# uzh-rpg/rpg_svo

Measured on AMD Instinct MI355X. Metric: frames/sec sparse-align+pose-refine (VGA, 4 pyr lvls); ATE vs CPU ref, higher is better.
Workload: dtype value = default build: K1 f32 pixels/residuals/chi2/per-pixel products, f64 Jacobian rows/partials/reductions/projection/solve/pose; K4 f64 (reference-width build: roofline_f64_build.value)

## Files before the change

### include/svo_hip.h

```cpp
#ifndef SVO_HIP_H_
#define SVO_HIP_H_

#include <stddef.h>
#include <stdint.h>

#ifdef __cplusplus
extern "C" {
#endif

#define SVO_HIP_MAX_LEVELS 8
#define SVO_HIP_STORE_TAIL_PAD 256
#define SVO_HIP_MAX_PATCHES 1024

#define SVO_HIP_OK 0
#define SVO_HIP_EINVAL (-1)
#define SVO_HIP_ERANGE (-2)
#define SVO_HIP_EHIP (-3)
#define SVO_HIP_ENODEV (-4)
#define SVO_HIP_ENOMEM (-5)

#define SVO_HIP_HALFSAMPLE_SCALAR 0
#define SVO_HIP_HALFSAMPLE_SSE2 1
#define SVO_HIP_HALFSAMPLE_AUTO 2

// ... 245 lines not shown
                                       double* d_px_cur, int32_t* d_ok, int32_t* d_ref_obs, int32_t* d_search_level,
                                       double* d_A_cur_ref, uint8_t* d_patch_out, void* d_workspace,
                                       size_t workspace_bytes, void* stream);
int svo_hip_select_matches_indirect(const svo_hip_camera* cam, int M_cap, const int32_t* d_M, const int32_t* d_cell,
                                    const int32_t* d_ok, const double* d_px, const int32_t* d_level,
                                    const double* d_pos, int max_fts, int32_t* d_n, int32_t* d_sel, double* d_f,
                                    int32_t* d_level_out, double* d_pos_out, uint8_t* d_has_point, int32_t* d_signal,
                                    int32_t signal_value, void* stream);

int svo_hip_compose_poses(int n, const double* d_A, const double* d_B, double* d_out,
                          const int32_t* d_out_index, void* stream);
int svo_hip_cam2world(const svo_hip_camera* cam, int n, const double* d_px, double* d_f,
                      void* stream);
int svo_hip_frame_pose_compose(const double* d_T_cur_ref, const double* d_q_ref, const double* d_t_ref, double* d_frame_T,
                               int cur_frame, double* d_T_copy, double* d_T_out, const svo_hip_camera* cam, int n_frames,
                               int n_kf, const double* d_key_pos, const uint8_t* d_key_valid, int max_n_kfs, int32_t* d_rank,
                               int32_t* d_rank_out, int32_t* d_signal, int32_t signal_value, void* stream);

int svo_hip_pose_optimize(const svo_hip_camera* cam, int B, const int32_t* d_n, int n_stride,
                          const double* d_f, const int32_t* d_level, const double* d_pos,
                          uint8_t* d_has_point, double reproj_thresh, int n_iter,
                          double* d_T_f_w, double* d_Cov, double* d_stats, int32_t* d_ran,
                          void* stream);
int svo_hip_pose_optimize_ordered(const svo_hip_camera* cam, int B, const int32_t* d_n, int n_stride,
                                  const double* d_f, const int32_t* d_level, const double* d_pos,
                                  uint8_t* d_has_point, double reproj_thresh, int n_iter,
                                  double* d_T_f_w, double* d_Cov, double* d_stats, int32_t* d_ran,
                                  void* stream);

int svo_hip_pose_optimize_deferred(const svo_hip_camera* cam, int B, const int32_t* d_n, int n_stride,
                                   const double* d_f, const int32_t* d_level, const double* d_pos,
                                   uint8_t* d_has_point, double reproj_thresh, int n_iter, double* d_T_f_w,
                                   double* d_Cov, double* d_stats, int32_t* d_ran, void* stream);

int svo_hip_point_optimize(const svo_hip_frames* frames, int P, const int32_t* d_obs_ptr,
                           const int32_t* d_obs_frame, const double* d_obs_f, int n_iter,
                           double* d_pos, void* stream);

typedef struct svo_hip_seeds {
  float* d_a;
  float* d_b;
  float* d_mu;
  float* d_z_range;
  float* d_sigma2;
  const int32_t* d_batch_id;
} svo_hip_seeds;

#define SVO_HIP_SEED_ERASED_OLD 1
#define SVO_HIP_SEED_BEHIND 2
#define SVO_HIP_SEED_NOT_IN_FRAME 3
#define SVO_HIP_SEED_NO_MATCH 4
#define SVO_HIP_SEED_UPDATED 5
#define SVO_HIP_SEED_CONVERGED 6
#define SVO_HIP_SEED_NAN 7

typedef struct svo_hip_depth_filter_options {
  int32_t max_n_kfs;
  int32_t batch_counter;
  double seed_convergence_sigma2_thresh;
  int32_t align_1d;
  int32_t align_max_iter;
  int32_t max_epi_search_steps;
  int32_t subpix_refinement;
  int32_t epi_search_edgelet_filtering;
  int32_t n_pyr_levels;
  double epi_search_edgelet_max_angle;
// ... 204 lines not shown
```

### rpg_svo_amd/capi.py

```python
from __future__ import annotations

import ctypes as C
import os

MAX_LEVELS = 8
STORE_TAIL_PAD = 256
MAX_PATCHES = 1024

HALFSAMPLE_SCALAR, HALFSAMPLE_SSE2, HALFSAMPLE_AUTO = 0, 1, 2
SIA_STOP = 1

_LIB_PATH = os.environ.get("SVO_HIP_LIB") or os.path.join(os.path.dirname(os.path.abspath(__file__)), "lib", "libsvo_hip.so")


class SvoHipError(RuntimeError):
    pass


class PyrLayout(C.Structure):
    _fields_ = [
        ("n_levels", C.c_int32),
        ("w", C.c_int32 * MAX_LEVELS),
        ("h", C.c_int32 * MAX_LEVELS),
        ("pitch", C.c_int32 * MAX_LEVELS),
# ... 176 lines not shown
    "svo_hip_sparse_align": (_i, [C.POINTER(PyrLayout), _vp, _i, _vp, _vp, _vp, _i, _vp, _vp, _vp,
                                  C.POINTER(SiaParams), _vp, _vp, _vp, _vp, _vp, _vp, _vp, _vp]),
    "svo_hip_sparse_align_workgroup": (_i, [C.POINTER(PyrLayout), _vp, _i, _vp, _vp, _vp, _i, _vp, _vp, _vp,
                                            C.POINTER(SiaParams), _vp, _vp, _vp, _vp, _vp, _vp, _vp, _vp]),
    "svo_hip_solve6_hipsolver_workspace_bytes": (C.c_size_t, [_i]),
    "svo_hip_solve6_hipsolver": (_i, [_i, _vp, _vp, _vp, _vp, _vp, C.c_size_t, _vp]),
    "svo_hip_align_batch": (_i, [_LP, _vp, _i, _vp, _vp, _vp, _vp, _vp, _i, _vp, _vp, _vp, _vp]),
    "svo_hip_align_batch_counted": (_i, [_LP, _vp, _i, _vp, _vp, _vp, _vp, _vp, _i, _vp, _vp, _vp, _vp, _vp]),
    "svo_hip_align_workspace_bytes": (C.c_size_t, [_i]),
    "svo_hip_align_batch_phased": (_i, [_LP, _vp, _i, _vp, _vp, _vp, _vp, _vp, _i, _vp, _vp, _vp, _vp, _vp, C.c_size_t, _vp]),
    "svo_hip_update_seeds_scan_steps": (_vp, [_vp]),
    "svo_hip_update_seeds_count_evaluations": (C.c_int, [C.c_int]),
    "svo_hip_update_seeds_align_evaluations": (_vp, [_vp, C.c_int]),
    "svo_hip_match_workspace_bytes": (C.c_size_t, [_i]),
    "svo_hip_find_match_direct": (_i, [_LP, _vp, C.POINTER(Camera), C.POINTER(Frames), _i, _vp, _vp, _vp,
                                       C.POINTER(Features), _i, _i, _vp, _vp, _vp, _vp, _vp, _vp, _vp, C.c_size_t, _vp]),
    "svo_hip_reproject_map": (_i, [C.POINTER(Camera), C.POINTER(Frames), _i, _vp, C.POINTER(Map), C.POINTER(MapPatch),
                                   C.POINTER(Grid), _i, _i, _i, _i, C.POINTER(Reprojection), _vp]),
    "svo_hip_find_match_direct_indirect": (_i, [_LP, _vp, C.POINTER(Camera), C.POINTER(Frames), _i, _vp, _vp, _vp, _vp, _vp,
                                                C.POINTER(Features), _i, _i, _vp, _vp, _vp, _vp, _vp, _vp, _vp, C.c_size_t, _vp]),
    "svo_hip_select_matches_indirect": (_i, [C.POINTER(Camera), _i, _vp, _vp, _vp, _vp, _vp, _vp, _i, _vp, _vp, _vp, _vp, _vp,
                                             _vp, _vp, _i, _vp]),
    "svo_hip_reproject_points": (_i, [C.POINTER(Camera), C.POINTER(Frames), _i, _vp, _vp, _i, _i, _vp, _vp, _vp]),
    "svo_hip_compose_poses": (_i, [_i, _vp, _vp, _vp, _vp, _vp]),
    "svo_hip_frame_pose_compose": (_i, [_vp, _vp, _vp, _vp, _i, _vp, _vp, _vp, _i, _i, _vp, _vp, _i, _vp, _vp, _vp, _i, _vp]),
    "svo_hip_cam2world": (_i, [C.POINTER(Camera), _i, _vp, _vp, _vp]),
    "svo_hip_select_matches": (_i, [C.POINTER(Camera), _i, _vp, _vp, _vp, _vp, _vp, _i, _vp, _vp, _vp, _vp, _vp, _vp, _vp, _i, _vp]),
    "svo_hip_pose_optimize": (_i, [C.POINTER(Camera), _i, _vp, _i, _vp, _vp, _vp, _vp, C.c_double, _i, _vp, _vp, _vp,
                                   _vp, _vp]),
    "svo_hip_pose_optimize_ordered": (_i, [C.POINTER(Camera), _i, _vp, _i, _vp, _vp, _vp, _vp, C.c_double, _i, _vp, _vp,
                                           _vp, _vp, _vp]),
    "svo_hip_pose_optimize_deferred": (_i, [C.POINTER(Camera), _i, _vp, _i, _vp, _vp, _vp, _vp, C.c_double, _i, _vp, _vp,
                                           _vp, _vp, _vp]),
    "svo_hip_point_optimize": (_i, [C.POINTER(Frames), _i, _vp, _vp, _vp, _i, _vp, _vp]),
    "svo_hip_update_seeds": (_i, [_LP, _vp, C.POINTER(Camera), C.POINTER(Frames), _i, _vp, C.POINTER(Features),
                                  C.POINTER(Seeds), C.POINTER(DepthFilterOptions), _vp, _vp, _vp, _vp, C.c_size_t, _vp]),
    "svo_hip_seed_store_patch": (_i, [C.POINTER(SeedPatch), C.POINTER(Features), C.POINTER(Seeds), _vp]),
    "svo_hip_update_seeds_resident": (_i, [_LP, _vp, C.POINTER(Camera), C.POINTER(Frames), _i, _i, _vp, C.POINTER(Features),
                                           C.POINTER(Seeds), C.POINTER(DepthFilterOptions), _vp, _vp, _vp, _vp, _vp, C.c_size_t, _vp]),
    "svo_hip_update_seeds_resident_pose": (_i, [_LP, _vp, C.POINTER(Camera), C.POINTER(Frames), _i, _vp, _i, _vp, C.POINTER(Features),
                                                C.POINTER(Seeds), C.POINTER(DepthFilterOptions), _vp, _vp, _vp, _vp, _vp, C.c_size_t, _vp]),
    "svo_hip_find_epipolar_match_direct": (_i, [_LP, _vp, C.POINTER(Camera), C.POINTER(Frames), _i, _vp, C.POINTER(Features),
                                                _vp, _vp, _vp, C.POINTER(DepthFilterOptions), _vp, _vp, _vp, _vp, _vp, C.c_size_t, _vp]),
    "svo_hip_update_seed_batch": (_i, [_i, _vp, _vp, C.POINTER(Seeds), _vp]),
    "svo_hip_fast_workspace_bytes": (C.c_size_t, [_LP, _i, _i]),
    "svo_hip_fast_detect": (_i, [_LP, _vp, _i, _vp, _i, _i, _i, _i, _i, _vp, C.c_double, _vp, _vp, _vp, _vp, C.c_size_t, _vp]),
    "svo_hip_klt_params_default": (_i, [C.POINTER(KltParams)]),
    "svo_hip_klt_track": (_i, [_LP, _vp, _i, _vp, _vp, _i, _vp, _vp, _vp, _vp, C.POINTER(KltParams), _vp]),
    "svo_hip_klt_summarize": (_i, [C.POINTER(Camera), _i, _i, _vp, _vp, _vp, _vp, _vp, _vp, _vp, _vp]),
    "svo_hip_homography_params_default": (_i, [C.POINTER(HomographyParams)]),
    "svo_hip_homography_init": (_i, [C.POINTER(Camera), _i, _i, _vp, _vp, _vp, _vp, _vp, _vp, C.POINTER(HomographyParams),
                                     C.POINTER(HomographyOut), _vp]),
    "svo_hip_first_map": (_i, [C.POINTER(Camera), _i, _i, _vp, _vp, _vp, _vp, _vp, _vp, _vp, _vp, _vp, _i, _i, _i, _i,
                               C.POINTER(FirstMapOut), _vp]),
    "svo_hip_initialize_seeds": (_i, [C.POINTER(Camera), _i, _i, _vp, _vp, _vp, C.c_double, _vp, _vp, _vp, _i, _i,
                                      C.POINTER(SeedInitOut), _vp]),
    "svo_hip_frame_close_params_default": (_i, [C.POINTER(FrameCloseParams)]),
    "svo_hip_frame_close": (_i, [C.POINTER(Camera), _i, _i, _i, C.POINTER(FrameCloseIn), _i, _i, _i, _i, C.POINTER(FrameCloseParams),
                                 C.POINTER(FrameCloseOut), _vp]),
    "svo_hip_compute_tau_batch": (_i, [_i, _vp, _vp, _vp, C.c_double, _vp, _vp]),
}

_lib = None


def lib_path() -> str:
# ... 54 lines not shown
```

### rpg_svo_amd/csrc/pose_optimizer.hip

```cpp
#pragma clang fp contract(off)
#include "track_kernels.h"
#include "track_math.h"

using namespace svo_capi;
using namespace svo_dev;

namespace {

constexpr int PO_MINW = 4;
constexpr int PO_HALF = 32;
constexpr int PO_BLOCK = 64;
constexpr int PO_MAXN = 1024;
constexpr double SVO_EPS = 0.0000000001;

struct PoseArgs {
  Cam cam;
  const int32_t* n;
  int n_stride;
  const double* f;
  const int32_t* level;
  const double* pos;
  uint8_t* has_point;
  double reproj_thresh;
  int n_iter;
  double* T;
  double* Cov;
  double* stats;
  int32_t* ran;
  int only_flagged;
};

struct PoseLds {
  double tile[28][PO_HALF];
  unsigned long long live[PO_BLOCK / 64];
  double acc[28];
  double dT[6];
  double new_chi2;
  Se3 T, T_old;
  double scale;
  double median_d;
  double chi2;
  float median_f;
  int n_err;
  int flag;
};

__device__ __forceinline__ float tukey_weight(float x) {
  const float b_square = 4.6851f * 4.6851f;
  const float x_square = x * x;
  if (x_square <= b_square) {
    const float tmp = 1.0f - x_square / b_square;
    return tmp * tmp;
  }
  return 0.0f;
}

template <typename T>
__device__ __forceinline__ void rank_select(const T* v, int n, int k, T* out) {
  for (int i = threadIdx.x; i < n; i += PO_BLOCK) {
    const T mine = v[i];
    if (!(mine < (T)INFINITY)) continue;
    int rank = 0;
#pragma unroll 8
    for (int j = 0; j < n; ++j) {
      const T o = v[j];
      rank += (o < mine || (o == mine && j < i)) ? 1 : 0;
    }
    if (rank == k) *out = mine;
  }
}

struct PoseDyn {
  double* vals;
  float* err;
  uint8_t* hp;
};

__global__ void __launch_bounds__(PO_BLOCK, PO_MINW) pose_opt_kernel(const PoseArgs a) {
  __shared__ PoseLds s;
  SVO_DYNAMIC_LDS(double, po_dyn);
  const int ns8 = (a.n_stride + 7) & ~7;
  PoseDyn d;
  d.vals = po_dyn;
  d.err = reinterpret_cast<float*>(po_dyn + ns8);
  d.hp = reinterpret_cast<uint8_t*>(d.err + ns8);
  const int b = blockIdx.x;
  const int tid = threadIdx.x;
  if (a.only_flagged && a.ran[b] != 2) return;
  int n = a.n[b];
  n = n < 0 ? 0 : (n > a.n_stride ? a.n_stride : n);
  const size_t base = (size_t)b * a.n_stride;
  const double focal = fabs(a.cam.fx);

  if (tid == 0) {
    se3_from_Rt(a.T + 12 * b, s.T);
    s.T_old = s.T;
    s.n_err = 0;
    s.flag = 0;
    s.chi2 = 0.0;
  }
  for (int i = tid; i < n; i += PO_BLOCK) d.hp[i] = a.has_point[base + i];
  __syncthreads();
  {
    const Se3 T = s.T;
    int cnt = 0;
    for (int i = tid; i < n; i += PO_BLOCK) {
      d.err[i] = INFINITY;
      if (!d.hp[i]) continue;
      const double p[3] = {a.pos[3 * (base + i)], a.pos[3 * (base + i) + 1], a.pos[3 * (base + i) + 2]};
      const double fb[3] = {a.f[3 * (base + i)], a.f[3 * (base + i) + 1], a.f[3 * (base + i) + 2]};
      double pf[3], u0[2], u1[2];
      se3_apply(T, p, pf);
      project2d(fb, u0);
      project2d(pf, u1);
      double e[2] = {u0[0] - u1[0], u0[1] - u1[1]};
      const double k = 1.0 / (double)(1 << a.level[base + i]);
      e[0] *= k;
      e[1] *= k;
      d.err[i] = (float)norm2(e);
      ++cnt;
    }
    if (cnt) atomicAdd(&s.n_err, cnt);
  }
  __syncthreads();
  const int n_err = s.n_err;
  if (n_err == 0) {
    if (tid == 0) a.ran[b] = 0;
    return;
  }
  rank_select<float>(d.err, n, n_err / 2, &s.median_f);
  __syncthreads();
  const double estimated_scale = (double)(1.48f * s.median_f);
  if (tid == 0) s.scale = estimated_scale;

  if (tid < 28) s.acc[tid] = 0.0;
  for (int iter = 0; iter < a.n_iter; ++iter) {
    if (tid == 0 && iter == 5) s.scale = 0.85 / focal;
    if (tid < 28) s.acc[tid] = 0.0;
    __syncthreads();
    const Se3 T = s.T;
    const double scale = s.scale;
    for (int c0 = 0; c0 < n; c0 += PO_BLOCK) {
      const int i = c0 + tid;
      double A21[21], bb[6], c2 = 0.0;
#pragma unroll
      for (int k = 0; k < 21; ++k) A21[k] = 0.0;
#pragma unroll
      for (int k = 0; k < 6; ++k) bb[k] = 0.0;
      bool live = false;
      if (i < n && d.hp[i]) {
        live = true;
        const double p[3] = {a.pos[3 * (base + i)], a.pos[3 * (base + i) + 1], a.pos[3 * (base + i) + 2]};
        const double fb[3] = {a.f[3 * (base + i)], a.f[3 * (base + i) + 1], a.f[3 * (base + i) + 2]};
        double J[12], xyz_f[3], u0[2], u1[2];
        se3_apply(T, p, xyz_f);
        frame_jacobian_xyz2uv(xyz_f, J);
        project2d(fb, u0);
        project2d(xyz_f, u1);
        double e[2] = {u0[0] - u1[0], u0[1] - u1[1]};
// ... 138 lines not shown
  const double reproj_thresh_scaled = a.reproj_thresh / focal;
  {
    const Se3 T = s.T;
    if (tid == 0) s.n_err = 0;
    __syncthreads();
    int deleted = 0;
    for (int i = tid; i < n; i += PO_BLOCK) {
      d.err[i] = 0.f;
      d.vals[i] = INFINITY;
      if (!d.hp[i]) continue;
      const double p[3] = {a.pos[3 * (base + i)], a.pos[3 * (base + i) + 1], a.pos[3 * (base + i) + 2]};
      const double fb[3] = {a.f[3 * (base + i)], a.f[3 * (base + i) + 1], a.f[3 * (base + i) + 2]};
      double pf[3], u0[2], u1[2];
      se3_apply(T, p, pf);
      project2d(fb, u0);
      project2d(pf, u1);
      double e[2] = {u0[0] - u1[0], u0[1] - u1[1]};
      const double k = 1.0 / (double)(1 << a.level[base + i]);
      e[0] *= k;
      e[1] *= k;
      d.vals[i] = e[0] * e[0] + e[1] * e[1];
      d.err[i] = 1.f;
      if (norm2(e) > reproj_thresh_scaled) {
        d.err[i] = 2.f;
        ++deleted;
      }
    }
    if (deleted) atomicAdd(&s.n_err, deleted);
  }
  __syncthreads();
  rank_select<double>(d.vals, n, n_err / 2, &s.median_d);
  __syncthreads();
  const int n_deleted = s.n_err;
  for (int i = tid; i < n; i += PO_BLOCK)
    if (d.err[i] == 2.f) a.has_point[base + i] = 0;
  if (tid == 0) {
    a.stats[4 * b + 0] = estimated_scale * focal;
    a.stats[4 * b + 1] = a.n_iter > 0 ? sqrt(med_init) * focal : 0.0;
    a.stats[4 * b + 2] = sqrt(s.median_d) * focal;
    a.stats[4 * b + 3] = (double)(n_err - n_deleted);
    a.ran[b] = 1;
  }
}

}

static int launch_ordered(const svo_track::PoseWaveArgs& w, int only_flagged, hipStream_t s) {
  PoseArgs a;
  a.cam = make_cam(&w.cam);
  a.n = w.n;
  a.n_stride = w.n_stride;
  a.f = w.f;
  a.level = w.level;
  a.pos = w.pos;
  a.has_point = w.has_point;
  a.reproj_thresh = w.reproj_thresh;
  a.n_iter = w.n_iter;
  a.T = w.T;
  a.Cov = w.Cov;
  a.stats = w.stats;
  a.ran = w.ran;
  a.only_flagged = only_flagged;
  const int ns8 = (w.n_stride + 7) & ~7;
  const size_t dyn = (size_t)ns8 * (sizeof(double) + sizeof(float) + 1);
  hipLaunchKernelGGL(pose_opt_kernel, dim3(w.B), dim3(PO_BLOCK), dyn, s, a);
  return check_launch();
}

enum PoseMode { POSE_WAVE_FINISH, POSE_WAVE_DEFERRED, POSE_ORDERED };

static int pose_optimize_impl(PoseMode mode, const svo_hip_camera* cam, int B, const int32_t* d_n, int n_stride, const double* d_f,
                              const int32_t* d_level, const double* d_pos, uint8_t* d_has_point, double reproj_thresh,
                              int n_iter, double* d_T_f_w, double* d_Cov, double* d_stats, int32_t* d_ran, void* stream) {
  if (!cam || !cam_model_ok(cam) || B < 0 || n_stride < 1 || n_iter < 0) return SVO_HIP_EINVAL;
  if (n_stride > PO_MAXN) return SVO_HIP_ERANGE;
  if (B == 0) return SVO_HIP_OK;
  if (!d_n || !d_f || !d_level || !d_pos || !d_has_point || !d_T_f_w || !d_stats || !d_ran) return SVO_HIP_EINVAL;
  svo_track::PoseWaveArgs w;
  w.cam = *cam;
  w.B = B;
  w.n = d_n;
  w.n_stride = n_stride;
  w.f = d_f;
  w.level = d_level;
  w.pos = d_pos;
  w.has_point = d_has_point;
  w.reproj_thresh = reproj_thresh;
  w.n_iter = n_iter;
  w.T = d_T_f_w;
  w.Cov = d_Cov;
  w.stats = d_stats;
  w.ran = d_ran;
  hipStream_t s = static_cast<hipStream_t>(stream);
  if (mode == POSE_ORDERED || n_stride > svo_track::POSE_WAVE_MAX_STRIDE)
    return launch_ordered(w, 0, s);
  const int rc = svo_track::launch_pose_wave(w, s);
  if (rc != SVO_HIP_OK || mode == POSE_WAVE_DEFERRED) return rc;
  return launch_ordered(w, 1, s);
}

extern "C" int svo_hip_pose_optimize(const svo_hip_camera* cam, int B, const int32_t* d_n, int n_stride,
                                     const double* d_f, const int32_t* d_level, const double* d_pos,
                                     uint8_t* d_has_point, double reproj_thresh, int n_iter, double* d_T_f_w,
                                     double* d_Cov, double* d_stats, int32_t* d_ran, void* stream) {
  return pose_optimize_impl(POSE_WAVE_FINISH, cam, B, d_n, n_stride, d_f, d_level, d_pos, d_has_point, reproj_thresh, n_iter, d_T_f_w,
                            d_Cov, d_stats, d_ran, stream);
}

extern "C" int svo_hip_pose_optimize_deferred(const svo_hip_camera* cam, int B, const int32_t* d_n, int n_stride,
                                              const double* d_f, const int32_t* d_level, const double* d_pos,
                                              uint8_t* d_has_point, double reproj_thresh, int n_iter, double* d_T_f_w,
                                              double* d_Cov, double* d_stats, int32_t* d_ran, void* stream) {
  return pose_optimize_impl(POSE_WAVE_DEFERRED, cam, B, d_n, n_stride, d_f, d_level, d_pos, d_has_point, reproj_thresh, n_iter, d_T_f_w,
                            d_Cov, d_stats, d_ran, stream);
}

extern "C" int svo_hip_pose_optimize_ordered(const svo_hip_camera* cam, int B, const int32_t* d_n, int n_stride,
                                             const double* d_f, const int32_t* d_level, const double* d_pos,
                                             uint8_t* d_has_point, double reproj_thresh, int n_iter, double* d_T_f_w,
                                             double* d_Cov, double* d_stats, int32_t* d_ran, void* stream) {
  return pose_optimize_impl(POSE_ORDERED, cam, B, d_n, n_stride, d_f, d_level, d_pos, d_has_point, reproj_thresh, n_iter, d_T_f_w,
                            d_Cov, d_stats, d_ran, stream);
}
```

### rpg_svo_amd/csrc/pose_optimizer_wave.hip

```cpp
#include "track_kernels.h"
#include "track_math.h"
#include "wave_reduce.h"

using namespace svo_capi;
using namespace svo_dev;

namespace {

using svo_track::PoseWaveArgs;

constexpr int PW_WAVES = 1;
constexpr int PW_MINW = 4;
constexpr double SVO_EPS = 0.0000000001;


__device__ __forceinline__ void uni_se3(Se3& T) {
#pragma unroll
  for (int k = 0; k < 4; ++k) T.q[k] = uniform_f64(T.q[k]);
#pragma unroll
  for (int k = 0; k < 3; ++k) T.t[k] = uniform_f64(T.t[k]);
}


__device__ __forceinline__ double wave_reduce32_f64(const double v[32], int lane) {
// ... 132 lines not shown
          }
        }
      }
      return found;
    }
  }
  return prefix;
}

__device__ __forceinline__ bool pivots_ok(const double A[21], const double LD[21]) {
  double dmax = 0.0, imax = 0.0;
  bool zero = false;
#pragma unroll
  for (int k = 0; k < 6; ++k) {
    dmax = fmax(dmax, fabs(A[sym6(k, k)]));
    const double id = fabs(LD[15 + k]);
    zero = zero || !(id > 0.0);
    imax = fmax(imax, id);
  }
  return !zero && (imax * dmax * 1e-9 < 1.0);
}

template <int J>
__device__ __forceinline__ double bcast(double v) { return readlane_f64<2 * J>(v); }

struct PwObs {
  double px, py, pz, ux, uy, k;
};

struct PwBlock {
  double* d;
  float* k;
  uint8_t* slot;
  int cap;
  __device__ __forceinline__ PwObs load(int c) const {
    PwObs o;
    o.px = d[c]; o.py = d[cap + c]; o.pz = d[2 * cap + c]; o.ux = d[3 * cap + c]; o.uy = d[4 * cap + c];
    o.k = (double)k[c];
    return o;
  }
};
constexpr int PW_BYTES_PER_OBS = 5 * 8 + 4 + 1;
__host__ __device__ constexpr int pw_cap(int n_stride) { return (n_stride + 7) & ~7; }

__device__ __forceinline__ double pw_e2(const PwObs& o, const double R[9], const double t[3]) {
  const double x = R[0] * o.px + R[1] * o.py + R[2] * o.pz + t[0];
  const double y = R[3] * o.px + R[4] * o.py + R[5] * o.pz + t[1];
  const double z = R[6] * o.px + R[7] * o.py + R[8] * o.pz + t[2];
  const double zi = fast_rcp(z);
  const double e0 = (o.ux - x * zi) * o.k, e1 = (o.uy - y * zi) * o.k;
  return e0 * e0 + e1 * e1;
}

__device__ __forceinline__ double pw_select(const unsigned long long kd[4], int trips, int k) {
  unsigned long long r;
  if (trips <= 1) r = radix_select<1, unsigned long long>(kd, k, 62);
  else if (trips == 2) r = radix_select<2, unsigned long long>(kd, k, 62);
  else if (trips == 3) r = radix_select<3, unsigned long long>(kd, k, 62);
  else r = radix_select<4, unsigned long long>(kd, k, 62);
  return __longlong_as_double((long long)r);
}

__global__ void __launch_bounds__(64 * PW_WAVES, PW_MINW) pose_opt_wave_kernel(const PoseWaveArgs a) {
  SVO_DYNAMIC_LDS(double, pw_dyn);
  const int lane = threadIdx.x & 63;
  const int wave = threadIdx.x >> 6;
  const int b = blockIdx.x * PW_WAVES + wave;
  if (b >= a.B) return;
  int n = __builtin_amdgcn_readfirstlane(a.n[b]);
  n = n < 0 ? 0 : (n > a.n_stride ? a.n_stride : n);
  const size_t base = (size_t)b * a.n_stride;
  const double focal = fabs(a.cam.fx);

  PwBlock blk;
  blk.cap = pw_cap(a.n_stride);
  blk.d = pw_dyn + (size_t)wave * (blk.cap / 8) * PW_BYTES_PER_OBS;
  blk.k = reinterpret_cast<float*>(blk.d + 5 * blk.cap);
  blk.slot = reinterpret_cast<uint8_t*>(blk.k + blk.cap);
  int n_live = 0;
  for (int j = 0; j * 64 < n; ++j) {
    const int i = j * 64 + lane;
    const bool live = (i < n) && a.has_point[base + i] != 0;
    const unsigned long long m = __ballot(live);
    if (live) {
      const int at = n_live + __popcll(m & ((1ull << lane) - 1ull));
      const int c = at < blk.cap ? at : blk.cap - 1;
      const double* p = a.pos + 3 * (base + i);
      const double* f = a.f + 3 * (base + i);
      blk.d[c] = p[0]; blk.d[blk.cap + c] = p[1]; blk.d[2 * blk.cap + c] = p[2];
      blk.d[3 * blk.cap + c] = f[0] / f[2];
      blk.d[4 * blk.cap + c] = f[1] / f[2];
      blk.k[c] = pow2_inv_f32(a.level[base + i]);
      blk.slot[c] = (uint8_t)i;
    }
    n_live += __popcll(m);
  }
  if (n_live == 0) {
    if (lane == 0) a.ran[b] = 0;
    return;
  }
  SVO_WAVE_LDS_FENCE();
  const int last_pos = (n_live < blk.cap ? n_live : blk.cap) - 1;
  const int trips = (n_live + 63) >> 6;

  Se3 T, T_old;
  se3_from_Rt(a.T + 12 * b, T);
  uni_se3(T);
  T_old = T;
  double R[9];
  quat_to_R(T.q, R);
#pragma unroll
  for (int k = 0; k < 9; ++k) R[k] = uniform_f64(R[k]);

  double estimated_scale, med_init;
  {
    unsigned long long kd[4];
#pragma unroll
    for (int j = 0; j < 4; ++j) {
      kd[j] = 0x7ff0000000000000ull;
      if (j < trips) {
        const int at = j * 64 + lane;
        const double e2 = pw_e2(blk.load(at < last_pos ? at : last_pos), R, T.t);
        if (at < n_live) kd[j] = (unsigned long long)__double_as_longlong(e2);
      }
    }
    med_init = pw_select(kd, trips, n_live / 2);
    const float median_f = (float)sqrt(med_init);
    estimated_scale = (double)(1.48f * median_f);
  }

  double scale = estimated_scale;
  double chi2 = 0.0;
  if (a.n_iter == 0) {
    if (lane == 0) a.ran[b] = 2;
    return;
  }
  for (int iter = 0; iter < a.n_iter; ++iter) {
    if (iter == 5) scale = 0.85 / focal;
    const double inv_scale = 1.0 / scale;
    double A[21];
    double acc[32];
#pragma unroll
    for (int k = 0; k < 32; ++k) acc[k] = 0.0;
#pragma unroll 1
    for (int j = 0; j < trips; ++j) {
      const int at = j * 64 + lane;
      const PwObs o = blk.load(at < last_pos ? at : last_pos);
      const double x = R[0] * o.px + R[1] * o.py + R[2] * o.pz + T.t[0];
      const double y = R[3] * o.px + R[4] * o.py + R[5] * o.pz + T.t[1];
      const double z = R[6] * o.px + R[7] * o.py + R[8] * o.pz + T.t[2];
      const double zi = fast_rcp(z);
      const double xn = x * zi, yn = y * zi;
      const double k = o.k;
      const double e0 = (o.ux - xn) * k, e1 = (o.uy - yn) * k;
      const double e2 = e0 * e0 + e1 * e1;
      const float wf = tukey_w((float)(fast_sqrt(e2) * inv_scale));
      const double w = at < n_live ? (double)wf : 0.0;
      const double j00 = -zi * k, j02 = xn * zi * k, j03 = xn * yn * k, j04 = -(1.0 + xn * xn) * k, j05 = yn * k;
      const double j12 = yn * zi * k, j13 = (1.0 + yn * yn) * k, j14 = -j03, j15 = -xn * k;
      const double w00 = w * j00, w02 = w * j02, w03 = w * j03, w04 = w * j04, w05 = w * j05;
      const double w11 = w00, w12 = w * j12, w13 = w * j13, w14 = w * j14, w15 = w * j15;
      acc[0] = fma(w00, j00, acc[0]);
      acc[1] = fma(w00, j02, acc[1]);
      acc[2] = fma(w00, j03, acc[2]);
      acc[3] = fma(w00, j04, acc[3]);
      acc[4] = fma(w00, j05, acc[4]);
      acc[6] = fma(w11, j12, acc[6]);
      acc[7] = fma(w11, j13, acc[7]);
      acc[9] = fma(w11, j15, acc[9]);
// ... 3 lines not shown
      acc[13] = fma(w02, j05, fma(w12, j15, acc[13]));
      acc[14] = fma(w03, j03, fma(w13, j13, acc[14]));
      acc[15] = fma(w03, j04, fma(w13, j14, acc[15]));
      acc[16] = fma(w03, j05, fma(w13, j15, acc[16]));
      acc[17] = fma(w04, j04, fma(w14, j14, acc[17]));
      acc[18] = fma(w04, j05, fma(w14, j15, acc[18]));
      acc[19] = fma(w05, j05, fma(w15, j15, acc[19]));
      acc[20] = fma(-w00, e0, acc[20]);
      acc[21] = fma(-w11, e1, acc[21]);
      acc[22] = fma(-w02, e0, fma(-w12, e1, acc[22]));
      acc[23] = fma(-w03, e0, fma(-w13, e1, acc[23]));
      acc[24] = fma(-w04, e0, fma(-w14, e1, acc[24]));
      acc[25] = fma(-w05, e0, fma(-w15, e1, acc[25]));
      acc[26] = fma(e2, w, acc[26]);
    }
    const double tot = wave_reduce32_f64(acc, lane);
    const double s0 = bcast<0>(tot), s1 = bcast<1>(tot), s2 = bcast<2>(tot), s3 = bcast<3>(tot), s4 = bcast<4>(tot);
    const double s6 = bcast<6>(tot), s7 = bcast<7>(tot), s9 = bcast<9>(tot);
    const double s10 = bcast<10>(tot), s11 = bcast<11>(tot), s12 = bcast<12>(tot), s13 = bcast<13>(tot);
    const double s14 = bcast<14>(tot), s15 = bcast<15>(tot), s16 = bcast<16>(tot), s17 = bcast<17>(tot);
    const double s18 = bcast<18>(tot), s19 = bcast<19>(tot);
    const double bv[6] = {bcast<20>(tot), bcast<21>(tot), bcast<22>(tot), bcast<23>(tot), bcast<24>(tot), bcast<25>(tot)};
    const double new_chi2 = bcast<26>(tot);
    A[sym6(0, 0)] = s0; A[sym6(0, 1)] = 0.0; A[sym6(0, 2)] = s1; A[sym6(0, 3)] = s2; A[sym6(0, 4)] = s3; A[sym6(0, 5)] = s4;
    A[sym6(1, 1)] = s0; A[sym6(1, 2)] = s6; A[sym6(1, 3)] = s7; A[sym6(1, 4)] = -s2; A[sym6(1, 5)] = s9;
    A[sym6(2, 2)] = s10; A[sym6(2, 3)] = s11; A[sym6(2, 4)] = s12; A[sym6(2, 5)] = s13;
    A[sym6(3, 3)] = s14; A[sym6(3, 4)] = s15; A[sym6(3, 5)] = s16;
    A[sym6(4, 4)] = s17; A[sym6(4, 5)] = s18; A[sym6(5, 5)] = s19;

    double dT[6];
    double LD[21];
    ldlt6_factor_fast(A, LD);
    if (!pivots_ok(A, LD)) {
      if (lane == 0) a.ran[b] = 2;
      return;
    }
    ldlt6_solve(LD, bv, dT);

    bool last = false;
    if ((iter > 0 && new_chi2 > chi2) || isnan(dT[0])) {
      T = T_old;
      last = true;
    } else {
      Se3 ex;
      se3_exp_fast(dT, ex.q, ex.t);
      T_old = T;
      T = se3_compose_fast(ex, T);
      uni_se3(T);
      chi2 = new_chi2;
      double nm = 0.0;
#pragma unroll
      for (int k = 0; k < 6; ++k) nm = fmax(nm, fabs(dT[k]));
      last = nm <= SVO_EPS;
    }
    quat_to_R(T.q, R);
#pragma unroll
    for (int k = 0; k < 9; ++k) R[k] = uniform_f64(R[k]);
    last = last || iter + 1 == a.n_iter;
    if (last) {
      if (a.Cov) {
        double e[6], x[6];
#pragma unroll
        for (int i = 0; i < 6; ++i) e[i] = (i == lane) ? 1.0 : 0.0;
        ldlt6_solve(LD, e, x);
        const double if2 = 1.0 / (focal * focal);
        if (lane < 6) {
#pragma unroll
          for (int i = 0; i < 6; ++i) a.Cov[36 * b + i * 6 + lane] = x[i] * if2;
        }
      }
      break;
    }
  }
  if (lane == 0) se3_to_Rt(T, a.T + 12 * b);

  const double reproj_thresh_scaled = a.reproj_thresh / focal;
  const double reproj_thresh2 = reproj_thresh_scaled * reproj_thresh_scaled;
  int n_deleted = 0;
  double med_final;
  {
    unsigned long long kd[4];
#pragma unroll
    for (int j = 0; j < 4; ++j) {
      kd[j] = 0x7ff0000000000000ull;
      if (j < trips) {
        const int at = j * 64 + lane;
        const int c = at < last_pos ? at : last_pos;
        const double e2 = pw_e2(blk.load(c), R, T.t);
        const bool live = at < n_live;
        if (live) kd[j] = (unsigned long long)__double_as_longlong(e2);
        const bool prune = live && e2 > reproj_thresh2;
        if (prune) {
          const int slot = blk.slot[c];
          if (slot < n) a.has_point[base + slot] = 0;
        }
        n_deleted += __popcll(__ballot(prune));
      }
    }
    med_final = pw_select(kd, trips, n_live / 2);
  }
  if (lane == 0) {
    a.stats[4 * b + 0] = estimated_scale * focal;
    a.stats[4 * b + 1] = a.n_iter > 0 ? sqrt(med_init) * focal : 0.0;
    a.stats[4 * b + 2] = sqrt(med_final) * focal;
    a.stats[4 * b + 3] = (double)(n_live - n_deleted);
    a.ran[b] = 1;
  }
}

}

namespace svo_track {

int launch_pose_wave(const PoseWaveArgs& a, hipStream_t s) {
  const int grid = (a.B + PW_WAVES - 1) / PW_WAVES;
  const size_t lds = (size_t)PW_WAVES * pw_cap(a.n_stride) * PW_BYTES_PER_OBS;
  hipLaunchKernelGGL(pose_opt_wave_kernel, dim3(grid), dim3(64 * PW_WAVES), lds, s, a);
  return check_launch();
}

}
```

### rpg_svo_amd/csrc/track_kernels.h

```cpp
#pragma once
#include "capi_common.h"

namespace svo_track {

struct AlignArgs {
  svo_hip_pyr_layout L;
  const uint8_t* store;
  int M;
  const int32_t* slot;
  const int32_t* level;
  const uint8_t* pwb;
  const float* dir;
  const uint8_t* use_1d;
  const uint8_t* active;
  int n_iter;
  const double* px_in;
  double* px_out;
  int scale_out;
  int32_t* ok;
  double* h_inv;
  int32_t* iters = nullptr;
  const int32_t* M_dev = nullptr;
  int it0 = 0, it1 = 1 << 30;
  const int32_t* queue_in = nullptr;
// ... 3 lines not shown
  int queue_cap = 0;
  float* state = nullptr;
};
constexpr int ALIGN_NQ = 64;
size_t align_phase_workspace_bytes(int M);
struct SeedArgs;
bool align_takes_finish(int M);
int launch_align(const AlignArgs& a, hipStream_t s, void* d_phase_ws = nullptr, size_t phase_ws_bytes = 0,
                 const SeedArgs* finish = nullptr);

struct WarpArgs {
  svo_hip_pyr_layout L;
  const uint8_t* store;
  int M;
  const uint8_t* active;
  const int32_t* ref_slot;
  const int32_t* ref_level;
  const int32_t* search_level;
  const float* A_ref_cur;
  const float* px_ref_pyr;
  uint8_t* pwb;
  const int32_t* M_dev = nullptr;
};
int launch_warp(const WarpArgs& a, hipStream_t s);

struct PoseWaveArgs {
  svo_hip_camera cam;
  int B;
  const int32_t* n;
  int n_stride;
  const double* f;
  const int32_t* level;
  const double* pos;
  uint8_t* has_point;
  double reproj_thresh;
  int n_iter;
  double* T;
  double* Cov;
  double* stats;
  int32_t* ran;
};
constexpr int POSE_WAVE_MAX_STRIDE = 256;
int launch_pose_wave(const PoseWaveArgs& a, hipStream_t s);

struct Carver {
  uint8_t* p;
  size_t left;
  bool ok = true;
  Carver(void* base, size_t bytes) : p(static_cast<uint8_t*>(base)), left(bytes) {}
  template <typename T>
  T* take(size_t n) {
    const size_t need = (n * sizeof(T) + 255) & ~size_t(255);
    if (need > left) { ok = false; return nullptr; }
    T* r = reinterpret_cast<T*>(p);
    p += need;
    left -= need;
    return r;
  }
  static size_t round(size_t n_bytes) { return (n_bytes + 255) & ~size_t(255); }
};

}
```

### rpg_svo_amd/tracking.py

```python
from __future__ import annotations

import ctypes as C
from dataclasses import dataclass

import torch

from . import capi
from .pyramid import PyramidStore, _stream_ptr


def _ptr(t):
    return None if t is None else t.data_ptr()


def _chk(t, dtype):
    assert t.is_cuda and t.dtype == dtype and t.is_contiguous(), "device-resident contiguous tensor required"
    return t


class FrameTable:

    def __init__(self, slot: torch.Tensor, T_f_w: torch.Tensor):
        self.slot = _chk(slot, torch.int32)
        self.T_f_w = _chk(T_f_w, torch.float64)
# ... 163 lines not shown
    dev = px.device
    cap = max(1, min(M, max_fts + 1))
    n = torch.zeros(1, dtype=torch.int32, device=dev)
    sel = torch.full((cap,), -1, dtype=torch.int32, device=dev)
    f = torch.zeros(cap, 3, dtype=torch.float64, device=dev)
    level_out = torch.zeros(cap, dtype=torch.int32, device=dev)
    pos_out = torch.zeros(cap, 3, dtype=torch.float64, device=dev)
    has_point = torch.zeros(cap, dtype=torch.uint8, device=dev)
    c = capi.camera(cam)
    capi.check(lib.svo_hip_select_matches(C.byref(c), M, _chk(cell, torch.int32).data_ptr(), _chk(ok, torch.int32).data_ptr(),
                                          _chk(px, torch.float64).data_ptr(), _chk(level, torch.int32).data_ptr(),
                                          _chk(pos, torch.float64).data_ptr(), int(max_fts), n.data_ptr(), sel.data_ptr(),
                                          f.data_ptr(), level_out.data_ptr(), pos_out.data_ptr(), has_point.data_ptr(),
                                          None, 0, _stream_ptr(dev)), "svo_hip_select_matches")
    return n, sel, f, level_out, pos_out, has_point


@dataclass
class PoseOptResult:
    T_f_w: torch.Tensor
    Cov: torch.Tensor
    stats: torch.Tensor
    ran: torch.Tensor
    has_point: torch.Tensor


def optimize_gauss_newton(cam, n, f, level, pos, has_point, T_f_w, reproj_thresh: float = 2.0, n_iter: int = 10,
                          ordered: bool = False, out: PoseOptResult | None = None, deferred: bool = False) -> PoseOptResult:
    lib = capi.load()
    B, ns = f.shape[0], f.shape[1]
    dev = f.device
    _chk(n, torch.int32); _chk(f, torch.float64); _chk(level, torch.int32); _chk(pos, torch.float64)
    _chk(has_point, torch.uint8); _chk(T_f_w, torch.float64)
    if out is not None:
        res = out
        res.T_f_w.copy_(T_f_w)
        res.has_point.copy_(has_point)
    else:
        res = PoseOptResult(T_f_w.clone(), torch.zeros(B, 36, dtype=torch.float64, device=dev),
                            torch.zeros(B, 4, dtype=torch.float64, device=dev), torch.zeros(B, dtype=torch.int32, device=dev),
                            has_point.clone())
    c = capi.camera(cam)
    fn = lib.svo_hip_pose_optimize_ordered if ordered else (lib.svo_hip_pose_optimize_deferred if deferred else lib.svo_hip_pose_optimize)
    capi.check(fn(C.byref(c), B, n.data_ptr(), ns, f.data_ptr(), level.data_ptr(), pos.data_ptr(),
                  res.has_point.data_ptr(), reproj_thresh, n_iter, res.T_f_w.data_ptr(),
                  res.Cov.data_ptr(), res.stats.data_ptr(), res.ran.data_ptr(), _stream_ptr(dev)),
               "svo_hip_pose_optimize")
    return res


@dataclass
class FrameClose:
    gate: torch.Tensor
    quality: torch.Tensor
    result: torch.Tensor
    T_out: torch.Tensor
    nobs_out: torch.Tensor
    depth_mean: torch.Tensor
    depth_min: torch.Tensor
    kf_block: torch.Tensor
    valid: torch.Tensor
    xyz_ref: torch.Tensor
    key_pts: torch.Tensor
    occupancy: torch.Tensor
    kf_remove: torch.Tensor


_FRAME_CLOSE_DTYPES = dict(gate=torch.int32, quality=torch.int32, result=torch.int32, T_out=torch.float64, nobs_out=torch.int32,
                           depth_mean=torch.float64, depth_min=torch.float64, kf_block=torch.int32, valid=torch.uint8,
                           xyz_ref=torch.float64, key_pts=torch.int32, occupancy=torch.uint8, kf_remove=torch.int32)


def frame_close_outputs(B: int, n_stride: int, cells: int, device) -> FrameClose:
    shape = dict(T_out=(B, 12), valid=(B, n_stride), xyz_ref=(B, n_stride, 3), key_pts=(B, 5), occupancy=(B, cells))
    return FrameClose(**{k: torch.zeros(shape.get(k, (B,)), dtype=dt, device=device) for k, dt in _FRAME_CLOSE_DTYPES.items()})
# ... 232 lines not shown
```

Before: 12.49 million.

## Add out-of-place pose optimize to drop host-side copies and chunk flagged fallback

Adds an out-of-place pose-optimization entry that reads the input pose and has_point row and writes the results directly to separate outputs. The Python wrapper no longer clones or copies them beforehand, which removes two device copy launches per call. The fallback kernel for flagged frames now launches one block per 64 frames and uses a ballot to gather only the flagged ones, instead of one block per frame that mostly exits at once. The cost is extra LDS per observation for the row buffer and writing the whole row for every frame.

```diff
diff --git a/include/svo_hip.h b/include/svo_hip.h
--- a/include/svo_hip.h
+++ b/include/svo_hip.h
@@ -301,6 +301,12 @@
                                    const double* d_f, const int32_t* d_level, const double* d_pos,
                                    uint8_t* d_has_point, double reproj_thresh, int n_iter, double* d_T_f_w,
                                    double* d_Cov, double* d_stats, int32_t* d_ran, void* stream);
+
+int svo_hip_pose_optimize_into(const svo_hip_camera* cam, int B, const int32_t* d_n, int n_stride,
+                               const double* d_f, const int32_t* d_level, const double* d_pos,
+                               const uint8_t* d_has_point_in, uint8_t* d_has_point_out, double reproj_thresh,
+                               int n_iter, const double* d_T_in, double* d_T_out, double* d_Cov, double* d_stats,
+                               int32_t* d_ran, void* stream);
 
 int svo_hip_point_optimize(const svo_hip_frames* frames, int P, const int32_t* d_obs_ptr,
                            const int32_t* d_obs_frame, const double* d_obs_f, int n_iter,
diff --git a/rpg_svo_amd/capi.py b/rpg_svo_amd/capi.py
--- a/rpg_svo_amd/capi.py
+++ b/rpg_svo_amd/capi.py
@@ -232,6 +232,8 @@
                                            _vp, _vp, _vp]),
     "svo_hip_pose_optimize_deferred": (_i, [C.POINTER(Camera), _i, _vp, _i, _vp, _vp, _vp, _vp, C.c_double, _i, _vp, _vp,
                                            _vp, _vp, _vp]),
+    "svo_hip_pose_optimize_into": (_i, [C.POINTER(Camera), _i, _vp, _i, _vp, _vp, _vp, _vp, _vp, C.c_double, _i, _vp, _vp,
+                                        _vp, _vp, _vp, _vp]),
     "svo_hip_point_optimize": (_i, [C.POINTER(Frames), _i, _vp, _vp, _vp, _i, _vp, _vp]),
     "svo_hip_update_seeds": (_i, [_LP, _vp, C.POINTER(Camera), C.POINTER(Frames), _i, _vp, C.POINTER(Features),
                                   C.POINTER(Seeds), C.POINTER(DepthFilterOptions), _vp, _vp, _vp, _vp, C.c_size_t, _vp]),
diff --git a/rpg_svo_amd/csrc/pose_optimizer.hip b/rpg_svo_amd/csrc/pose_optimizer.hip
--- a/rpg_svo_amd/csrc/pose_optimizer.hip
+++ b/rpg_svo_amd/csrc/pose_optimizer.hip
@@ -20,14 +20,16 @@
   const double* f;
   const int32_t* level;
   const double* pos;
+  const uint8_t* has_point_in;
   uint8_t* has_point;
   double reproj_thresh;
   int n_iter;
+  const double* T_in;
   double* T;
   double* Cov;
   double* stats;
   int32_t* ran;
-  int only_flagged;
+  int B;
 };
 
 struct PoseLds {
@@ -76,30 +78,24 @@
   uint8_t* hp;
 };
 
-__global__ void __launch_bounds__(PO_BLOCK, PO_MINW) pose_opt_kernel(const PoseArgs a) {
-  __shared__ PoseLds s;
-  SVO_DYNAMIC_LDS(double, po_dyn);
-  const int ns8 = (a.n_stride + 7) & ~7;
-  PoseDyn d;
-  d.vals = po_dyn;
-  d.err = reinterpret_cast<float*>(po_dyn + ns8);
-  d.hp = reinterpret_cast<uint8_t*>(d.err + ns8);
-  const int b = blockIdx.x;
+__device__ __forceinline__ bool po_row_out(const PoseArgs& a) { return a.has_point != a.has_point_in; }
+
+__device__ __forceinline__ void pose_opt_frame(const PoseArgs& a, const int b, PoseLds& s, const PoseDyn& d) {
   const int tid = threadIdx.x;
-  if (a.only_flagged && a.ran[b] != 2) return;
   int n = a.n[b];
   n = n < 0 ? 0 : (n > a.n_stride ? a.n_stride : n);
   const size_t base = (size_t)b * a.n_stride;
   const double focal = fabs(a.cam.fx);
+  const int n_row = po_row_out(a) ? a.n_stride : n;
 
   if (tid == 0) {
-    se3_from_Rt(a.T + 12 * b, s.T);
+    se3_from_Rt(a.T_in + 12 * b, s.T);
     s.T_old = s.T;
     s.n_err = 0;
     s.flag = 0;
     s.chi2 = 0.0;
   }
-  for (int i = tid; i < n; i += PO_BLOCK) d.hp[i] = a.has_point[base + i];
+  for (int i = tid; i < n_row; i += PO_BLOCK) d.hp[i] = a.has_point_in[base + i];
   __syncthreads();
   {
     const Se3 T = s.T;
@@ -125,6 +121,9 @@
   __syncthreads();
   const int n_err = s.n_err;
   if (n_err == 0) {
+    if (po_row_out(a))
+      for (int i = tid; i < n_row; i += PO_BLOCK) a.has_point[base + i] = d.hp[i];
+    if (a.T != a.T_in && tid < 12) a.T[12 * b + tid] = a.T_in[12 * b + tid];
     if (tid == 0) a.ran[b] = 0;
     return;
   }
@@ -329,14 +328,47 @@
   rank_select<double>(d.vals, n, n_err / 2, &s.median_d);
   __syncthreads();
   const int n_deleted = s.n_err;
-  for (int i = tid; i < n; i += PO_BLOCK)
-    if (d.err[i] == 2.f) a.has_point[base + i] = 0;
+  if (po_row_out(a)) {
+    for (int i = tid; i < n_row; i += PO_BLOCK) a.has_point[base + i] = (i < n && d.err[i] == 2.f) ? (uint8_t)0 : d.hp[i];
+  } else {
+    for (int i = tid; i < n; i += PO_BLOCK)
+      if (d.err[i] == 2.f) a.has_point[base + i] = 0;
+  }
   if (tid == 0) {
     a.stats[4 * b + 0] = estimated_scale * focal;
     a.stats[4 * b + 1] = a.n_iter > 0 ? sqrt(med_init) * focal : 0.0;
     a.stats[4 * b + 2] = sqrt(s.median_d) * focal;
     a.stats[4 * b + 3] = (double)(n_err - n_deleted);
     a.ran[b] = 1;
+  }
+}
+
+template <bool CHUNKED>
+__global__ void __launch_bounds__(PO_BLOCK, PO_MINW) pose_opt_kernel(const PoseArgs a) {
+  __shared__ PoseLds s;
+  SVO_DYNAMIC_LDS(double, po_dyn);
+  const int ns8 = (a.n_stride + 7) & ~7;
+  PoseDyn d;
+  d.vals = po_dyn;
+  d.err = reinterpret_cast<float*>(po_dyn + ns8);
+  d.hp = reinterpret_cast<uint8_t*>(d.err + ns8);
+  if (!CHUNKED) {
+    pose_opt_frame(a, blockIdx.x, s, d);
+    return;
+  }
+  static_assert(PO_BLOCK == 64, "one ballot covers the chunk");
+  __shared__ int todo[PO_BLOCK];
+  const int tid = threadIdx.x;
+  const int mine = blockIdx.x * PO_BLOCK + tid;
+  const bool flagged = mine < a.B && a.ran[mine] == 2;
+  const unsigned long long m = __ballot(flagged);
+  if (m == 0) return;
+  if (flagged) todo[__popcll(m & ((1ull << tid) - 1ull))] = mine;
+  const int n_todo = __popcll(m);
+  __syncthreads();
+  for (int k = 0; k < n_todo; ++k) {
+    pose_opt_frame(a, __builtin_amdgcn_readfirstlane(todo[k]), s, d);
+    __syncthreads();
   }
 }
 
@@ -350,29 +382,44 @@
   a.f = w.f;
   a.level = w.level;
   a.pos = w.pos;
+  a.has_point_in = w.has_point_in;
   a.has_point = w.has_point;
   a.reproj_thresh = w.reproj_thresh;
   a.n_iter = w.n_iter;
+  a.T_in = w.T_in;
   a.T = w.T;
   a.Cov = w.Cov;
   a.stats = w.stats;
   a.ran = w.ran;
-  a.only_flagged = only_flagged;
+  a.B = w.B;
   const int ns8 = (w.n_stride + 7) & ~7;
   const size_t dyn = (size_t)ns8 * (sizeof(double) + sizeof(float) + 1);
-  hipLaunchKernelGGL(pose_opt_kernel, dim3(w.B), dim3(PO_BLOCK), dyn, s, a);
+  if (only_flagged) {
+    hipLaunchKernelGGL(pose_opt_kernel<true>, dim3((w.B + PO_BLOCK - 1) / PO_BLOCK), dim3(PO_BLOCK), dyn, s, a);
+  } else {
+    hipLaunchKernelGGL(pose_opt_kernel<false>, dim3(w.B), dim3(PO_BLOCK), dyn, s, a);
+  }
   return check_launch();
 }
 
 enum PoseMode { POSE_WAVE_FINISH, POSE_WAVE_DEFERRED, POSE_ORDERED };
 
+static bool overlap_in_part(const void* p, const void* q, size_t bytes) {
+  const uintptr_t a = reinterpret_cast<uintptr_t>(p), b = reinterpret_cast<uintptr_t>(q);
+  return a != b && (a < b ? b - a : a - b) < bytes;
+}
+
 static int pose_optimize_impl(PoseMode mode, const svo_hip_camera* cam, int B, const int32_t* d_n, int n_stride, const double* d_f,
-                              const int32_t* d_level, const double* d_pos, uint8_t* d_has_point, double reproj_thresh,
-                              int n_iter, double* d_T_f_w, double* d_Cov, double* d_stats, int32_t* d_ran, void* stream) {
+                              const int32_t* d_level, const double* d_pos, const uint8_t* d_has_point_in, uint8_t* d_has_point,
+                              double reproj_thresh, int n_iter, const double* d_T_in, double* d_T_f_w, double* d_Cov, double* d_stats,
+                              int32_t* d_ran, void* stream) {
   if (!cam || !cam_model_ok(cam) || B < 0 || n_stride < 1 || n_iter < 0) return SVO_HIP_EINVAL;
   if (n_stride > PO_MAXN) return SVO_HIP_ERANGE;
   if (B == 0) return SVO_HIP_OK;
-  if (!d_n || !d_f || !d_level || !d_pos || !d_has_point || !d_T_f_w || !d_stats || !d_ran) return SVO_HIP_EINVAL;
+  if (!d_n || !d_f || !d_level || !d_pos || !d_has_point_in || !d_has_point || !d_T_in || !d_T_f_w || !d_stats || !d_ran)
+    return SVO_HIP_EINVAL;
+  if (overlap_in_part(d_has_point_in, d_has_point, (size_t)B * n_stride) || overlap_in_part(d_T_in, d_T_f_w, (size_t)B * 12 * sizeof(double)))
+    return SVO_HIP_EINVAL;
   svo_track::PoseWaveArgs w;
   w.cam = *cam;
   w.B = B;
@@ -381,9 +428,11 @@
   w.f = d_f;
   w.level = d_level;
   w.pos = d_pos;
+  w.has_point_in = d_has_point_in;
   w.has_point = d_has_point;
   w.reproj_thresh = reproj_thresh;
   w.n_iter = n_iter;
+  w.T_in = d_T_in;
   w.T = d_T_f_w;
   w.Cov = d_Cov;
   w.stats = d_stats;
@@ -396,26 +445,35 @@
   return launch_ordered(w, 1, s);
 }
 
+extern "C" int svo_hip_pose_optimize_into(const svo_hip_camera* cam, int B, const int32_t* d_n, int n_stride,
+                                          const double* d_f, const int32_t* d_level, const double* d_pos,
+                                          const uint8_t* d_has_point_in, uint8_t* d_has_point_out, double reproj_thresh,
+                                          int n_iter, const double* d_T_in, double* d_T_out, double* d_Cov, double* d_stats,
+                                          int32_t* d_ran, void* stream) {
+  return pose_optimize_impl(POSE_WAVE_FINISH, cam, B, d_n, n_stride, d_f, d_level, d_pos, d_has_point_in, d_has_point_out, reproj_thresh,
+                            n_iter, d_T_in, d_T_out, d_Cov, d_stats, d_ran, stream);
+}
+
 extern "C" int svo_hip_pose_optimize(const svo_hip_camera* cam, int B, const int32_t* d_n, int n_stride,
                                      const double* d_f, const int32_t* d_level, const double* d_pos,
                                      uint8_t* d_has_point, double reproj_thresh, int n_iter, double* d_T_f_w,
                                      double* d_Cov, double* d_stats, int32_t* d_ran, void* stream) {
-  return pose_optimize_impl(POSE_WAVE_FINISH, cam, B, d_n, n_stride, d_f, d_level, d_pos, d_has_point, reproj_thresh, n_iter, d_T_f_w,
-                            d_Cov, d_stats, d_ran, stream);
+  return pose_optimize_impl(POSE_WAVE_FINISH, cam, B, d_n, n_stride, d_f, d_level, d_pos, d_has_point, d_has_point, reproj_thresh, n_iter,
+                            d_T_f_w, d_T_f_w, d_Cov, d_stats, d_ran, stream);
 }
 
 extern "C" int svo_hip_pose_optimize_deferred(const svo_hip_camera* cam, int B, const int32_t* d_n, int n_stride,
                                               const double* d_f, const int32_t* d_level, const double* d_pos,
                                               uint8_t* d_has_point, double reproj_thresh, int n_iter, double* d_T_f_w,
                                               double* d_Cov, double* d_stats, int32_t* d_ran, void* stream) {
-  return pose_optimize_impl(POSE_WAVE_DEFERRED, cam, B, d_n, n_stride, d_f, d_level, d_pos, d_has_point, reproj_thresh, n_iter, d_T_f_w,
-                            d_Cov, d_stats, d_ran, stream);
+  return pose_optimize_impl(POSE_WAVE_DEFERRED, cam, B, d_n, n_stride, d_f, d_level, d_pos, d_has_point, d_has_point, reproj_thresh, n_iter,
+                            d_T_f_w, d_T_f_w, d_Cov, d_stats, d_ran, stream);
 }
 
 extern "C" int svo_hip_pose_optimize_ordered(const svo_hip_camera* cam, int B, const int32_t* d_n, int n_stride,
                                              const double* d_f, const int32_t* d_level, const double* d_pos,
                                              uint8_t* d_has_point, double reproj_thresh, int n_iter, double* d_T_f_w,
                                              double* d_Cov, double* d_stats, int32_t* d_ran, void* stream) {
-  return pose_optimize_impl(POSE_ORDERED, cam, B, d_n, n_stride, d_f, d_level, d_pos, d_has_point, reproj_thresh, n_iter, d_T_f_w,
-                            d_Cov, d_stats, d_ran, stream);
-}
+  return pose_optimize_impl(POSE_ORDERED, cam, B, d_n, n_stride, d_f, d_level, d_pos, d_has_point, d_has_point, reproj_thresh, n_iter,
+                            d_T_f_w, d_T_f_w, d_Cov, d_stats, d_ran, stream);
+}
diff --git a/rpg_svo_amd/csrc/pose_optimizer_wave.hip b/rpg_svo_amd/csrc/pose_optimizer_wave.hip
--- a/rpg_svo_amd/csrc/pose_optimizer_wave.hip
+++ b/rpg_svo_amd/csrc/pose_optimizer_wave.hip
@@ -188,6 +188,7 @@
   double* d;
   float* k;
   uint8_t* slot;
+  uint8_t* row;
   int cap;
   __device__ __forceinline__ PwObs load(int c) const {
     PwObs o;
@@ -196,8 +197,25 @@
     return o;
   }
 };
-constexpr int PW_BYTES_PER_OBS = 5 * 8 + 4 + 1;
+constexpr int PW_BYTES_PER_OBS = 5 * 8 + 4 + 1 + 1;
 __host__ __device__ constexpr int pw_cap(int n_stride) { return (n_stride + 7) & ~7; }
+
+__device__ __forceinline__ bool pw_row_out(const PoseWaveArgs& a) { return a.has_point != a.has_point_in; }
+__device__ __forceinline__ bool pw_pose_out(const PoseWaveArgs& a) { return a.T != a.T_in; }
+
+__device__ __forceinline__ void pw_store_row(const PoseWaveArgs& a, const uint8_t* row, int b, int lane) {
+  uint8_t* out = a.has_point + (size_t)b * a.n_stride;
+  if (((reinterpret_cast<uintptr_t>(out) | (unsigned)a.n_stride) & 3u) == 0) {
+    for (int i = lane; 4 * i < a.n_stride; i += 64) reinterpret_cast<uint32_t*>(out)[i] = reinterpret_cast<const uint32_t*>(row)[i];
+  } else {
+    for (int i = lane; i < a.n_stride; i += 64) out[i] = row[i];
+  }
+}
+
+__device__ __forceinline__ void pw_leave_untouched(const PoseWaveArgs& a, const uint8_t* row, int b, int lane) {
+  if (pw_row_out(a)) pw_store_row(a, row, b, lane);
+  if (pw_pose_out(a) && lane < 12) a.T[12 * b + lane] = a.T_in[12 * b + lane];
+}
 
 __device__ __forceinline__ double pw_e2(const PwObs& o, const double R[9], const double t[3]) {
   const double x = R[0] * o.px + R[1] * o.py + R[2] * o.pz + t[0];
@@ -233,10 +251,14 @@
   blk.d = pw_dyn + (size_t)wave * (blk.cap / 8) * PW_BYTES_PER_OBS;
   blk.k = reinterpret_cast<float*>(blk.d + 5 * blk.cap);
   blk.slot = reinterpret_cast<uint8_t*>(blk.k + blk.cap);
+  blk.row = blk.slot + blk.cap;
+  const int n_row = pw_row_out(a) ? a.n_stride : n;
   int n_live = 0;
-  for (int j = 0; j * 64 < n; ++j) {
+  for (int j = 0; j * 64 < n_row; ++j) {
     const int i = j * 64 + lane;
-    const bool live = (i < n) && a.has_point[base + i] != 0;
+    const uint8_t flag = i < n_row ? a.has_point_in[base + i] : (uint8_t)0;
+    if (pw_row_out(a) && i < n_row) blk.row[i] = flag;
+    const bool live = (i < n) && flag != 0;
     const unsigned long long m = __ballot(live);
     if (live) {
       const int at = n_live + __popcll(m & ((1ull << lane) - 1ull));
@@ -251,16 +273,17 @@
     }
     n_live += __popcll(m);
   }
+  SVO_WAVE_LDS_FENCE();
   if (n_live == 0) {
+    pw_leave_untouched(a, blk.row, b, lane);
     if (lane == 0) a.ran[b] = 0;
     return;
   }
-  SVO_WAVE_LDS_FENCE();
   const int last_pos = (n_live < blk.cap ? n_live : blk.cap) - 1;
   const int trips = (n_live + 63) >> 6;
 
   Se3 T, T_old;
-  se3_from_Rt(a.T + 12 * b, T);
+  se3_from_Rt(a.T_in + 12 * b, T);
   uni_se3(T);
   T_old = T;
   double R[9];
@@ -287,10 +310,7 @@
 
   double scale = estimated_scale;
   double chi2 = 0.0;
-  if (a.n_iter == 0) {
-    if (lane == 0) a.ran[b] = 2;
-    return;
-  }
+  bool handed_over = a.n_iter == 0;
   for (int iter = 0; iter < a.n_iter; ++iter) {
     if (iter == 5) scale = 0.85 / focal;
     const double inv_scale = 1.0 / scale;
@@ -360,8 +380,8 @@
     double LD[21];
     ldlt6_factor_fast(A, LD);
     if (!pivots_ok(A, LD)) {
-      if (lane == 0) a.ran[b] = 2;
-      return;
+      handed_over = true;
+      break;
     }
     ldlt6_solve(LD, bv, dT);
 
@@ -400,6 +420,11 @@
       break;
     }
   }
+  if (handed_over) {
+    pw_leave_untouched(a, blk.row, b, lane);
+    if (lane == 0) a.ran[b] = 2;
+    return;
+  }
   if (lane == 0) se3_to_Rt(T, a.T + 12 * b);
 
   const double reproj_thresh_scaled = a.reproj_thresh / focal;
@@ -420,12 +445,19 @@
         const bool prune = live && e2 > reproj_thresh2;
         if (prune) {
           const int slot = blk.slot[c];
-          if (slot < n) a.has_point[base + slot] = 0;
+          if (slot < n) {
+            if (pw_row_out(a)) blk.row[slot] = 0;
+            else a.has_point[base + slot] = 0;
+          }
         }
         n_deleted += __popcll(__ballot(prune));
       }
     }
     med_final = pw_select(kd, trips, n_live / 2);
+  }
+  if (pw_row_out(a)) {
+    SVO_WAVE_LDS_FENCE();
+    pw_store_row(a, blk.row, b, lane);
   }
   if (lane == 0) {
     a.stats[4 * b + 0] = estimated_scale * focal;
diff --git a/rpg_svo_amd/csrc/track_kernels.h b/rpg_svo_amd/csrc/track_kernels.h
--- a/rpg_svo_amd/csrc/track_kernels.h
+++ b/rpg_svo_amd/csrc/track_kernels.h
@@ -59,9 +59,11 @@
   const double* f;
   const int32_t* level;
   const double* pos;
+  const uint8_t* has_point_in;
   uint8_t* has_point;
   double reproj_thresh;
   int n_iter;
+  const double* T_in;
   double* T;
   double* Cov;
   double* stats;
diff --git a/rpg_svo_amd/tracking.py b/rpg_svo_amd/tracking.py
--- a/rpg_svo_amd/tracking.py
+++ b/rpg_svo_amd/tracking.py
@@ -219,15 +219,24 @@
     dev = f.device
     _chk(n, torch.int32); _chk(f, torch.float64); _chk(level, torch.int32); _chk(pos, torch.float64)
     _chk(has_point, torch.uint8); _chk(T_f_w, torch.float64)
+    into = not (ordered or deferred)
     if out is not None:
         res = out
-        res.T_f_w.copy_(T_f_w)
-        res.has_point.copy_(has_point)
+        if not into:
+            res.T_f_w.copy_(T_f_w)
+            res.has_point.copy_(has_point)
     else:
-        res = PoseOptResult(T_f_w.clone(), torch.zeros(B, 36, dtype=torch.float64, device=dev),
+        res = PoseOptResult(torch.empty_like(T_f_w) if into else T_f_w.clone(), torch.zeros(B, 36, dtype=torch.float64, device=dev),
                             torch.zeros(B, 4, dtype=torch.float64, device=dev), torch.zeros(B, dtype=torch.int32, device=dev),
-                            has_point.clone())
+                            torch.empty_like(has_point) if into else has_point.clone())
     c = capi.camera(cam)
+    if into:
+        _chk(res.T_f_w, torch.float64); _chk(res.has_point, torch.uint8)
+        capi.check(lib.svo_hip_pose_optimize_into(C.byref(c), B, n.data_ptr(), ns, f.data_ptr(), level.data_ptr(), pos.data_ptr(),
+                                                  has_point.data_ptr(), res.has_point.data_ptr(), reproj_thresh, n_iter,
+                                                  T_f_w.data_ptr(), res.T_f_w.data_ptr(), res.Cov.data_ptr(), res.stats.data_ptr(),
+                                                  res.ran.data_ptr(), _stream_ptr(dev)), "svo_hip_pose_optimize_into")
+        return res
     fn = lib.svo_hip_pose_optimize_ordered if ordered else (lib.svo_hip_pose_optimize_deferred if deferred else lib.svo_hip_pose_optimize)
     capi.check(fn(C.byref(c), B, n.data_ptr(), ns, f.data_ptr(), level.data_ptr(), pos.data_ptr(),
                   res.has_point.data_ptr(), reproj_thresh, n_iter, res.T_f_w.data_ptr(),
```

After: 12.55 million, median of 6. About the same (+0.5%).
